# shubhamchandak94/Spring

Hardware: AMD Instinct MI355X
Metric: Mreads/s through reorder stage (higher is better)
Workload: dtype u64; 1 GPU; 100000000 x 150 bp single-end synthetic reads per GPU (uniform genome 600000000 bp, 25x coverage, 1.0% substitutions, 50% reverse-complemented), inputs resident in HBM as .dna records; reads_per_gpu=100000000, read_len=150, chains=65536, num_thr=8, parallelism=single GPU, unmatched=13958636, singletons=12720853, rounds=1984, chain_groups=2

## Files before the change

### __graft_entry__.py

```python
import os
import sys

ROOT = os.path.dirname(os.path.abspath(__file__))
for p in (ROOT, os.path.join(ROOT, "tests")):
    if p not in sys.path:
        sys.path.insert(0, p)


def build():
    from spring_amd import build as b
    lib = b.build()
    assert os.path.exists(lib)
    from oracle import pyoracle
    pyoracle.build()
    import spring_amd
    from spring_amd import _lib
    _lib.lib()


def smoke():
    import numpy as np
    import spring_amd
    from oracle import pyoracle as po
    n, L = 20000, 100
    dna = spring_amd.synth_dna_host(n, L, n * L // 25, 1, 10000)
    read, ln = po.load_dna(dna, n, L)
    for K, fused, A, PH, KA, want in ((1, 0, 1, 1, 0, po.reorder_serial(read, ln, L)), (64, 0, 1, 1, 0, po.reorder_rounds(read, ln, L, 64, 2)),
                                  (64, 3, 1, 1, 0, po.reorder_rounds(read, ln, L, 64, 2)), (64, 3, 1, 1, -1, po.reorder_rounds(read, ln, L, 64, 2)),
                                  (64, 0, 2, 1, 0, po.reorder_rounds(read, ln, L, 64, 2, alternatives=2)),
                                  (4096, 3, 1, 2, 0, po.reorder_rounds_ph(read, ln, L, 4096, 2))):
        got = spring_amd.reorder_dna(dna, n, L, spring_amd.ReorderOpts(device=0, num_chains=K, num_thr=1 if K == 1 else 2, fused=fused,
                                                                       alternatives=A, phases=PH, known_absent=KA))
        for k in ("order", "rc", "flag", "pos", "rlen", "order_s"):
            assert np.array_equal(got[k], want[k]), (K, fused, A, PH, KA, k)
    from spring_amd.encoder import EncoderStage
    with spring_amd.ReorderStage(spring_amd.ReorderOpts(device=0, num_chains=64, num_thr=2, fused=3, alternatives=1, phases=1)) as st:
        st.load_dna(dna, n, L)
        st.run()
        streams = st.streams()
        with EncoderStage(0) as enc:
            enc.encode(st)
            got = enc.streams()
    want = po.encode(read, ln, L, streams, num_thr=2)
    for k in ("seq", "pos", "noise", "noisepos", "order", "rlen", "rc", "unaligned"):
        a, b = got[k], want[k]
        assert (a == b) if isinstance(a, bytes) else np.array_equal(a, b), ("encoder", k)
    print("smoke OK: %d reads, K=1, K=64 (both round kernels) and two chain groups bit-exact vs oracle; encoder stage bit-exact (%d contigs)"
          % (n, got["num_contigs"]))


if __name__ == "__main__":
    build()
    if "--smoke" in sys.argv:
        smoke()
```

### include/spring_reorder.h

```cpp
#ifndef SPRING_REORDER_H_
#define SPRING_REORDER_H_

#include <stddef.h>
#include <stdint.h>

#ifdef __cplusplus
extern "C" {
#endif

#define SPRING_REORDER_E_ARG (-1)
#define SPRING_REORDER_E_IO (-2)
#define SPRING_REORDER_E_HIP (-3)
#define SPRING_REORDER_E_STATE (-4)

typedef struct spring_reorder_ctx spring_reorder_ctx;

typedef struct {
  int32_t device;
  uint32_t num_chains;
  int32_t num_thr;
  int32_t collect_stats;
  int32_t time_search;
  int32_t force_literal_update;
  int32_t rounds_per_sync;
// ... 2 lines not shown
  int32_t seed_wide;
  int32_t tab_scale;
  int32_t search_wpb;
  int32_t dbg_search_lds;
  int32_t dbg_apply_lds;
  int32_t fused;
  int32_t deep_bins;
  int32_t num_devices;
  int32_t devices[8];
  int32_t mg_host_transport;
  int32_t table_mode;
  int32_t plan0[6];
  int32_t plan1[6];
  int32_t long_min;
  int32_t long_blocks;
  int32_t debug;
  int32_t long_split;
  int32_t entry_flags;
  int32_t out_writers;
  int32_t alternatives;
  int32_t phases;
  int32_t known_absent;
  int32_t sort_prefix_bits;
} spring_reorder_opts;

typedef struct {
  uint64_t n_reads, n_matched, n_single, unmatched;
  uint64_t probes, keyok, cands, hits, iterations, rounds, lost;
  uint64_t numkeys[2], dict_numreads[2];
  double ms_unpack, ms_dict, ms_chains, ms_finalize, ms_total;
  double ms_search_kernel;
  uint64_t search_launches;
  uint64_t device_bytes;
  double ms_exchange, ms_resolve_mark;
  uint64_t chains;
  uint64_t deep_pool;
  uint64_t long_searches;
  uint64_t table_minz;
  uint64_t table_marked_lines;
  uint64_t long_splits;
  uint64_t alternatives;
  uint64_t phases;
  double ms_search_busy;
  uint64_t sort_prefix_bits;
  uint64_t sort_repaired_runs;
  uint64_t sort_full_sorts;
  uint64_t sort_long_runs;
  uint64_t sort_list_overflows;
} spring_reorder_stats;

void spring_reorder_default_opts(spring_reorder_opts *o);
const char *spring_reorder_last_error(void);
void spring_reorder_trim_pool(void);

int spring_reorder_run(const char *temp_dir, uint32_t max_readlen, int32_t num_thr, int32_t paired_end,
                       uint32_t num_reads_clean_0, uint32_t num_reads_clean_1,
                       const spring_reorder_opts *opts );

int spring_reorder_create(spring_reorder_ctx **ctx, const spring_reorder_opts *opts);
void spring_reorder_destroy(spring_reorder_ctx *ctx);

int spring_reorder_load_dna(spring_reorder_ctx *ctx, const uint8_t *dna, size_t nbytes, uint32_t n,
                            uint32_t max_readlen);

int spring_reorder_load_dna_device(spring_reorder_ctx *ctx, const void *d_dna, size_t nbytes, uint32_t n,
                                   uint32_t max_readlen, int32_t fixed_len);

int spring_reorder_build_dict(spring_reorder_ctx *ctx);

int spring_reorder_run_chains(spring_reorder_ctx *ctx);
int spring_reorder_auto_chains(spring_reorder_ctx *ctx, uint32_t *chains, int32_t *deep);
// ... 74 lines not shown
```

### spring_amd/_lib.py

```python
import ctypes as C
import os

HERE = os.path.dirname(os.path.abspath(__file__))
LIB_PATH = os.environ.get("SPRING_AMD_LIB") or os.path.join(HERE, "lib", "libspring_reorder_hip.so")

EXPORTS = [
    "spring_reorder_default_opts", "spring_reorder_last_error", "spring_reorder_trim_pool", "spring_reorder_run", "spring_reorder_create",
    "spring_reorder_destroy", "spring_reorder_load_dna", "spring_reorder_load_dna_device",
    "spring_reorder_build_dict", "spring_reorder_run_chains", "spring_reorder_auto_chains", "spring_reorder_finalize",
    "spring_reorder_mg_begin", "spring_reorder_mg_search", "spring_reorder_mg_slice", "spring_reorder_mg_slices",
    "spring_reorder_mg_apply",
    "spring_reorder_mg_end", "spring_reorder_mg_exchange_virtual", "spring_reorder_debug_check_seed_state",
    "spring_mg_rccl_unique_id", "spring_mg_comm_create_rccl", "spring_mg_comm_create_host", "spring_mg_comm_destroy",
    "spring_reorder_mg_run",
    "spring_reorder_get_stats", "spring_reorder_download", "spring_reorder_tid_split", "spring_reorder_emit_dna",
    "spring_reorder_dict_lookup", "spring_reorder_download_reads", "spring_synth_dna_bytes",
    "spring_reorder_load_fastq", "spring_reorder_fastq_N",
    "spring_order_invert_se", "spring_order_invert_pe", "spring_order_correct", "spring_order_pe_encode",
    "spring_fastq_reorder",
    "spring_synth_dna_host", "spring_synth_genome_host", "spring_synth_dna_device", "spring_reorder_load_synth", "spring_reorder_download_dna",
    "spring_encoder_create", "spring_encoder_destroy", "spring_encoder_set_split_tables", "spring_encoder_encode_reorder", "spring_encoder_download",
    "spring_encoder_download_seq_packed", "spring_encoder_get_info", "spring_reorder_encode_run", "spring_encoder_encode_host", "spring_encoder_run",
]

# ... 1 lines not shown
    "spring_streams_create", "spring_streams_destroy", "spring_streams_from_encoder", "spring_streams_from_host",
    "spring_streams_download", "spring_streams_get_info", "spring_streams_run",
]
STREAMS_NUM = 9

DECODE_EXPORTS = [
    "spring_decode_create", "spring_decode_destroy", "spring_decode_seq_from_encoder", "spring_decode_seq_from_host",
    "spring_decode_seq_from_files", "spring_decode_from_streams", "spring_decode_from_host", "spring_decode_from_files",
    "spring_decode_download", "spring_decode_get_info",
]


class Opts(C.Structure):
    _fields_ = [("device", C.c_int32), ("num_chains", C.c_uint32), ("num_thr", C.c_int32),
                ("collect_stats", C.c_int32), ("time_search", C.c_int32), ("force_literal_update", C.c_int32),
                ("rounds_per_sync", C.c_int32), ("long_budget", C.c_int32),
                ("first_shifts", C.c_int32), ("seed_wide", C.c_int32), ("tab_scale", C.c_int32),
                ("search_wpb", C.c_int32), ("dbg_search_lds", C.c_int32), ("dbg_apply_lds", C.c_int32),
                ("fused", C.c_int32), ("deep_bins", C.c_int32),
                ("num_devices", C.c_int32), ("devices", C.c_int32 * 8), ("mg_host_transport", C.c_int32),
                ("table_mode", C.c_int32), ("plan0", C.c_int32 * 6), ("plan1", C.c_int32 * 6), ("long_min", C.c_int32),
                ("long_blocks", C.c_int32), ("debug", C.c_int32), ("long_split", C.c_int32), ("entry_flags", C.c_int32),
                ("out_writers", C.c_int32), ("alternatives", C.c_int32), ("phases", C.c_int32), ("known_absent", C.c_int32),
                ("sort_prefix_bits", C.c_int32)]


class FastqInfo(C.Structure):
    _fields_ = [("num_reads", C.c_uint32 * 2), ("num_reads_clean", C.c_uint32 * 2), ("num_reads_N", C.c_uint32 * 2),
                ("max_readlen", C.c_uint32), ("pad", C.c_uint32), ("ms_device", C.c_double)]


class EncoderInfo(C.Structure):
    _fields_ = ([(k, C.c_uint64) for k in ("n_aligned", "n_total", "seq_len", "noise_bytes", "n_noisepos",
                                           "unaligned_bytes", "len_unaligned", "num_contigs")]
                + [(k, C.c_uint32) for k in ("matched_s", "matched_N", "align_passes", "max_bin")]
                + [("ms_device", C.c_double), ("ms_phase", C.c_double * 8)])

    def asdict(self):
        d = {}
        for k, _ in self._fields_:
            v = getattr(self, k)
            d[k] = list(v) if hasattr(v, "__len__") else v
        return d


class StreamsInfo(C.Structure):
    _fields_ = ([("num_units", C.c_uint64), ("num_blocks", C.c_uint64), ("bytes", C.c_uint64 * STREAMS_NUM),
# ... 14 lines not shown
                + [(k, C.c_uint64) for k in ("n_aligned", "n_unaligned", "pos_escapes")]
                + [("ms_device", C.c_double), ("ms_file", C.c_double)])

    def asdict(self):
        d = {}
        for k, _ in self._fields_:
            v = getattr(self, k)
            d[k] = list(v) if hasattr(v, "__len__") else v
        return d


class Stats(C.Structure):
    _fields_ = ([(k, C.c_uint64) for k in ("n_reads", "n_matched", "n_single", "unmatched", "probes", "keyok",
                                          "cands", "hits", "iterations", "rounds", "lost")]
                + [("numkeys", C.c_uint64 * 2), ("dict_numreads", C.c_uint64 * 2)]
                + [(k, C.c_double) for k in ("ms_unpack", "ms_dict", "ms_chains", "ms_finalize", "ms_total",
                                             "ms_search_kernel")]
                + [("search_launches", C.c_uint64), ("device_bytes", C.c_uint64),
                   ("ms_exchange", C.c_double), ("ms_resolve_mark", C.c_double), ("chains", C.c_uint64),
                   ("deep_pool", C.c_uint64), ("long_searches", C.c_uint64),
                   ("table_minz", C.c_uint64), ("table_marked_lines", C.c_uint64), ("long_splits", C.c_uint64), ("alternatives", C.c_uint64), ("phases", C.c_uint64),
                   ("ms_search_busy", C.c_double),
                   ("sort_prefix_bits", C.c_uint64), ("sort_repaired_runs", C.c_uint64), ("sort_full_sorts", C.c_uint64),
                   ("sort_long_runs", C.c_uint64), ("sort_list_overflows", C.c_uint64)])

    def asdict(self):
        d = {}
        for k, _ in self._fields_:
            v = getattr(self, k)
            d[k] = list(v) if hasattr(v, "__len__") else v
        return d


MG_ALLGATHER_FN = C.CFUNCTYPE(C.c_int, C.c_void_p, C.c_size_t, C.c_size_t, C.c_size_t, C.c_void_p)

_lib = None


def lib():
    global _lib
    if _lib is not None:
        return _lib
    if not os.path.exists(LIB_PATH):
        raise RuntimeError(
            "spring_amd: %s is missing. Build it with `python -m spring_amd.build` "
            "(or __graft_entry__.build()); there is no CPU fallback." % LIB_PATH)
    L = C.CDLL(LIB_PATH)
# ... 103 lines not shown
```

### spring_amd/csrc/reorder_device.h

```cpp
#ifndef SPRING_REORDER_DEVICE_H_
#define SPRING_REORDER_DEVICE_H_

#include <hip/hip_runtime.h>
#include <stdint.h>

namespace sr {

constexpr int MAX_READ_LEN = 511;
constexpr int MAX_SEARCH = 1000;
constexpr int THRESH = 4;
constexpr uint32_t DEEP_BIN = 16;
constexpr uint32_t MID_BIN = 64;
constexpr uint32_t BIG_BIN = 256;
constexpr uint32_t CHUNK = 64;
constexpr uint32_t MARK_BLOCK = 256;
constexpr uint32_t MC_WAVES_PER_BLOCK = MARK_BLOCK / 4 + 3;
constexpr int UBLK_SHIFT = 12;
constexpr int LDS_PAD = 10;
constexpr int LDS_LIMBS = 16 + 2 * LDS_PAD;

enum { MODE_SEARCH = 0, MODE_NEED_SEED = 1 };
enum { PROP_NONE = 0, PROP_MATCH = 1, PROP_SEED = 2, PROP_FRESH = 3  };
enum { PK_NONE = 0, PK_MATCH = 1, PK_SEED = 2, PK_NOSEED = 4, PK_DONE = 5 };
constexpr unsigned long long PK_CURSOR_BIT = 1ull << 35;
constexpr unsigned long long PK_WILLNEED_BIT = 1ull << 36;
constexpr int PK_ALT_SHIFT = 37;
constexpr uint32_t ALT_MAX_READS = (1u << 27) - 1;
constexpr uint32_t ALT_KEY = 1u << 28;

struct __attribute__((aligned(16))) ChainHot {
  long long ref_pos;
  int32_t ref_len;
  uint32_t e_slot;
  uint32_t prev, first_rid;
  uint32_t n_emit, n_single;
  uint32_t s_slot;
  uint32_t num_reads_thr, num_unmatched_past;
  uint32_t prop_rid;
  union {
    struct {
      uint32_t done : 1, prev_unmatched : 1, left_search : 1, stop_searching : 1;
      uint32_t mode : 1, retrying : 1, finishing : 1, cursor_writer : 1;
      uint32_t cnt_buf : 1;
      uint32_t cnt_wide : 1;
      uint32_t prop_kind : 2;
      uint32_t prop_rev : 3;
      uint32_t prop_shift : 9;
    };
    uint32_t flags;
  };
  uint32_t alt1;
  uint32_t pad[2];
};
static_assert(sizeof(ChainHot) == 64, "ChainHot must be one 64-byte line");

struct __attribute__((aligned(64))) Chain {
  ChainHot h;
  uint64_t ref[16];
  uint64_t revref[16];
  uint64_t st_probes, st_keyok, st_cands, st_iter, st_lost, st_hits, n_unmatched, st_long ;
#ifdef SR_PHASE_TIMING
  uint64_t pt[64];
#endif
};
#ifndef SR_PHASE_TIMING
static_assert(sizeof(Chain) == 384, "Chain layout");
#endif

struct Globals {
  long long cursor;
  uint32_t alive;
  uint32_t e_alloc;
  uint32_t s_alloc;
  uint32_t pad;
  long long cursor_b;
};

struct TabView {
  const uint4 *buck;
  int bshift;
  int minz;
  int lshift;
};
// ... 19 lines not shown
  int plan[2][6];
  int seed_wide;
  int deep_bins;
  int search_wpb;
  int dbg_search_lds, dbg_apply_lds;
  int wl;
  int dstart[2], dend[2];
  uint32_t numkeys[2];
  TabView tab;
  const ulonglong2 *urec[2];
  const uint32_t *ids[2];
  uint32_t *epos[2];
  uint32_t idmask;
  const ulonglong2 *sig[2];
  uint64_t *taken;
  uint32_t *ublk;
  uint32_t *resv;
  uint32_t *needy;
  uint32_t *needy_cnt;
  uint32_t *needy_cnt_next;
  int fused;
  int alts;
  int mc;
  int ka, ka_lo;
  uint32_t *ord;
  uint4 *ord_cnt;
  uint32_t *longq;
  int long_budget, long_min, long_blocks, long_part;
  uint32_t *lctl, *lparts;
  struct LongHead *lhead;
  uint2 *lbin;
  uint16_t *lbcode;
  uint32_t lbin_stride;
#ifdef SR_PHASE_TIMING
  unsigned long long *dbg;
#endif
  Globals *glob;
  long long *cursor;
  uint32_t K, c0, Ktot;
  int phases;
  uint32_t g0, Kg, g0_other, Kg_other;
  uint32_t gg0, gKg, gKg_other;
  uint32_t seed_lo, seed_hi;
  uint32_t nb_lo, nb_hi;
  const uint64_t *taken_other;
  uint32_t *won, *won_other;
// ... 90 lines not shown
```

### spring_amd/csrc/reorder_kernels.hip

```cpp
#include <cstdlib>
#include <cstring>
#include <hip/hip_runtime.h>
#include <rocprim/rocprim.hpp>

#include "reorder_device.h"
#include "synth_common.h"

namespace sr {


__device__ __forceinline__ uint64_t mix64(uint64_t x) {
  x ^= x >> 33; x *= 0xff51afd7ed558ccdull; x ^= x >> 33; x *= 0xc4ceb9fe1a85ec53ull; x ^= x >> 33;
  return x;
}

__device__ __forceinline__ void wave_sync() {
  __builtin_amdgcn_fence(__ATOMIC_SEQ_CST, "wavefront");
  __builtin_amdgcn_wave_barrier();
}

__device__ __forceinline__ int uni_i32(int v) { return __builtin_amdgcn_readfirstlane(v); }
template <class T>
__device__ __forceinline__ T *uni_ptr(T *p) {
  const uint64_t a = reinterpret_cast<uint64_t>(p);
// ... 798 lines not shown
  WaveLds *ws = &lds[wave];
  const uint32_t step = P.n / P.Ktot;
  const uint32_t seed = cid * step;
  const bool start = P.n > 0 && (cid == 0 || step > 0);
  ChainHot h;
  memset(&h, 0, sizeof(h));
  if (lane == 0) {
    P.e_chunk[li] = make_uint2(li, 0u);
    P.s_chunk[li] = make_uint2(li, 0u);
  }
  if (!start) {
    h.done = 1;
    store_hot(c, h, lane);
    if (lane == 0 && P.prop) P.prop[cid] = (unsigned long long)PK_DONE << 32;
    return;
  }
  const int n = P.uniform_len ? P.L : (int)P.lens[seed];
  bool ovf0;
  const int Rn = wave_update_compute<NP, false>(P, li, ws, nullptr, seed, n, true, false, 0, 0, 0, false, false, ovf0, lane);
  pack_consensus(ws, Rn, lane, c);
  h.prev = seed; h.first_rid = seed; h.prev_unmatched = 1;
  h.e_slot = li * CHUNK; h.s_slot = li * CHUNK;
  h.ref_len = Rn; h.cnt_buf = 1; h.cnt_wide = 0;
  if (P.fused) h.prop_kind = PROP_FRESH;
  store_hot(c, h, lane);
  if (lane == 0) {
    c->n_unmatched = 1;
    if (P.prop) P.prop[cid] = (unsigned long long)PK_NONE << 32;
  }
}
__device__ __forceinline__ void mark_dead(const DevParams &P, uint32_t rid) {
#pragma unroll
  for (int l = 0; l < 2; l++) {
    if (!P.epos[l]) continue;
    const uint32_t e = P.epos[l][rid];
    if (e != 0xffffffffu) atomicOr(const_cast<uint32_t *>(P.ids[l]) + e, 0x80000000u);
  }
}
__global__ void k_build_epos(const uint32_t *__restrict__ ids, uint64_t m, uint32_t *__restrict__ epos) {
  const uint64_t i = (uint64_t)blockIdx.x * blockDim.x + threadIdx.x;
  if (i < m) epos[ids[i]] = (uint32_t)i;
}
void launch_build_epos(hipStream_t st, const uint32_t *ids, uint64_t m, uint32_t *epos) {
  if (m) hipLaunchKernelGGL(k_build_epos, dim3((unsigned)((m + 255) / 256)), dim3(256), 0, st, ids, m, epos);
}
__global__ void k_init_seeds(DevParams P) {
// ... 1736 lines not shown
}
__global__ void k_delay(uint32_t us) {
  const uint64_t t0 = wall_clock64();
  while (wall_clock64() - t0 < (uint64_t)us * 100u) __builtin_amdgcn_s_sleep(64);
}
__global__ void k_init_ord(DevParams P) {
  const uint32_t cid = P.gg0 + blockIdx.x * blockDim.x + threadIdx.x;
  const uint32_t blk = P.gg0 / MARK_BLOCK + blockIdx.x;
  __shared__ uint32_t s_n;
  if (threadIdx.x == 0) s_n = 0;
  __syncthreads();
  const bool local = cid < P.gg0 + P.gKg && cid - P.c0 - P.g0 < P.Kg;
  const uint64_t m = __ballot(local);
  uint32_t wbase = 0;
  if ((threadIdx.x & 63) == 0 && m) wbase = atomicAdd(&s_n, (uint32_t)__popcll(m));
  wbase = (uint32_t)__shfl((int)wbase, 0, 64);
  if (local) P.ord[(size_t)blk * MARK_BLOCK + wbase + (uint32_t)__popcll(m & ((1ull << (threadIdx.x & 63)) - 1))] = cid - P.c0;
  __syncthreads();
  if (threadIdx.x == 0) P.ord_cnt[blk] = make_uint4(0u, 0u, s_n, 0u);
}

__global__ void k_chain_summary(DevParams P, uint2 *__restrict__ sum, unsigned long long *__restrict__ tot ) {
  const uint32_t i = blockIdx.x * blockDim.x + threadIdx.x;
  uint64_t v[8] = {0, 0, 0, 0, 0, 0, 0, 0};
  if (i < P.K) {
    const Chain &c = P.chains[i];
    sum[i] = make_uint2(c.h.n_emit, c.h.n_single);
    v[0] = c.n_unmatched; v[1] = c.st_probes; v[2] = c.st_keyok; v[3] = c.st_cands; v[4] = c.st_iter; v[5] = c.st_lost; v[6] = c.st_hits; v[7] = c.st_long;
  }
#pragma unroll
  for (int k = 0; k < 8; k++) {
    const uint64_t w = wave_sum_u64(v[k]);
    if ((threadIdx.x & 63) == 0 && w) atomicAdd(&tot[k], (unsigned long long)w);
  }
}

__global__ void k_scatter_matched(DevParams P, uint64_t cap, const uint64_t *__restrict__ off_m) {
  uint64_t i = (uint64_t)blockIdx.x * blockDim.x + threadIdx.x;
  if (i >= cap) return;
  const uint2 ci = P.e_chunk[i / CHUNK];
  if (ci.x == 0xffffffffu) return;
  const uint32_t seq = ci.y + (uint32_t)(i % CHUNK);
  if (seq >= P.chains[ci.x].h.n_emit) return;
  const uint4 r = P.e_rec[i];
  const uint64_t d = off_m[ci.x] + seq;
  P.f_order[d] = r.x; P.f_rc[d] = (char)(r.y & 0xffu); P.f_flag[d] = (char)((r.y >> 8) & 0xffu);
  P.f_pos[d] = (long long)((unsigned long long)r.z | ((unsigned long long)r.w << 32));
  P.f_len[d] = P.uniform_len ? (uint16_t)P.L : P.lens[r.x];
}
__global__ void k_scatter_single(DevParams P, uint64_t cap, const uint64_t *__restrict__ off_s) {
  uint64_t i = (uint64_t)blockIdx.x * blockDim.x + threadIdx.x;
  if (i >= cap) return;
  const uint2 ci = P.s_chunk[i / CHUNK];
  if (ci.x == 0xffffffffu) return;
// ... 370 lines not shown
```

### spring_amd/csrc/reorder_pipeline.cpp

```cpp
#include <hip/hip_runtime.h>
#include <dlfcn.h>

#include <algorithm>
#include <system_error>
#include <thread>
#include <memory>
#include <atomic>
#include <chrono>
#include <cstdarg>
#include <cstdio>
#include <cstdlib>
#include <cstring>
#include <map>
#include <mutex>
#include <new>
#include <stdexcept>
#include <string>
#include <unordered_map>
#include <vector>
#include <zlib.h>

#include "reorder_device.h"
#include "reorder_internal.h"
#include "spring_reorder.h"
// ... 1388 lines not shown
  DMALLOC(P.cnt8, (size_t)K * 2 * ctx->Lpad * sizeof(uint32_t) + 64);
  const size_t cap = (size_t)n + (size_t)K * CHUNK;
  if (cap > 0xfffffff0ull) return fail(SPRING_REORDER_E_ARG, "n + K*%u exceeds the 32-bit slot space", CHUNK);
  ctx->cap = cap;
  const size_t nchunk = cap / CHUNK + 2;
  DMALLOC(P.e_rec, cap * sizeof(uint4)); DMALLOC(P.e_chunk, nchunk * sizeof(uint2));
  DMALLOC(P.s_rec, cap * 4); DMALLOC(P.s_chunk, nchunk * sizeof(uint2));
  P.mc = ctx->o.fused == 2 ? 0 : 1;
  bool ka_ok = false;
  int ka_lo = 0;
  if (P.Lpad <= 192 && ctx->o.known_absent >= 0 && !ctx->minz) {
    const int wlen = ctx->dict[0].end - ctx->dict[0].start + 1, lo = ctx->dict[0].start >> 5;
    if (wlen <= 32 && ctx->dict[1].start == ctx->dict[0].end + 1 && ctx->dict[1].end - ctx->dict[1].start + 1 == wlen &&
        2 * (ctx->L - wlen) + 2 <= 64 * (lo + 4) && 2 * ctx->dict[1].start + 2 <= 256 && lo + 4 <= 6) {
      ka_ok = true; ka_lo = lo;
    }
  }
  const uint64_t nd_ = (uint64_t)ctx->dict[0].numreads + ctx->dict[1].numreads, nk_ = (uint64_t)ctx->dict[0].numkeys + ctx->dict[1].numkeys;
  const uint32_t mc_min = P.phases == 2 ? ((ka_ok && nd_ * 100 < nk_ * 105) ? 20480u : 32768u) : 49152u;
  if (K < mc_min && ctx->o.fused != 3) P.mc = 0;
  if (64 - ctx->bshift > 32) P.mc = 0;
  P.ka = (P.mc && ka_ok) ? 1 : 0;
  P.ka_lo = P.ka ? ka_lo : 0;
  if (ctx->minz && !(fused && P.mc && !ctx->o.collect_stats && !P.deep_bins))
    return fail(SPRING_REORDER_E_ARG, "table_mode = 2 (minimizer-addressed table) is an experiment of the four-chain round kernel: "
                "shallow dictionary, at least 49152 chains or fused = 3, no work counters");
  if (!P.mc && !P.deep_bins && ctx->o.first_shifts == 0 && !ctx->user_plan0) {
    memset(P.plan[0], 0, sizeof(P.plan[0]));
    P.plan[0][0] = 8; P.plan[0][1] = 16;
  }
  P.g0 = 0; P.Kg = K; P.g0_other = 0; P.Kg_other = 0;
  P.gg0 = 0; P.gKg = Ktot; P.gKg_other = 0;
  P.seed_lo = 0; P.seed_hi = n;
  P.nb_lo = 0; P.nb_hi = (Ktot + 2047) / 2048;
  P.taken_other = nullptr; P.won = P.won_other = nullptr;
  ctx->taken2 = nullptr; ctx->resv2 = nullptr; ctx->won = nullptr;
  ctx->lb2 = spring_reorder_ctx::LongBufs();
  if (P.phases == 2) {
    DMALLOC(ctx->taken2, nwords * 8);
    DMALLOC(ctx->resv2, nn * 4);
    DMALLOC(ctx->won, (size_t)Ktot * 4);
  }
  P.prop = nullptr; P.alive_wave = nullptr; P.needy_cnt = P.needy_cnt_next = nullptr;
  ctx->cnt_buf[0] = ctx->cnt_buf[1] = nullptr;
  if (fused && P.deep_bins && ctx->o.entry_flags >= 0 && n < 0x80000000u) {
    for (int l = 0; l < 2; l++) {
// ... 827 lines not shown
    ctx->stats.ms_search_kernel = ms_round; ctx->stats.ms_search_busy = ms_round; ctx->stats.search_launches = timed_rounds;
    ctx->stats.ms_exchange = ms_xchg; ctx->stats.ms_resolve_mark = ms_mark;
  }
  if (ret) {
    const std::string keep = g_err;
    (void)hipStreamSynchronize(st);
    (void)spring_reorder_mg_end(ctx);
    g_err = keep;
    return ret;
  }
  return spring_reorder_mg_end(ctx);
}

int spring_reorder_finalize(spring_reorder_ctx *ctx) {
  if (!ctx) return fail(SPRING_REORDER_E_ARG, "ctx is NULL");
  if (ctx->stage != ST_CHAINS) return fail(SPRING_REORDER_E_STATE, "finalize: run_chains first");
  HIPCHK(hipSetDevice(ctx->dev));
  hipStream_t st = ctx->st;
  DevParams &P = ctx->P;
  const uint32_t K = ctx->K;
  const int T = ctx->o.num_thr;
  HIPCHK(hipEventRecord(ctx->ev[6], st));
  std::vector<uint2> hs(std::max<uint32_t>(K, 1));
  unsigned long long htot[8] = {0, 0, 0, 0, 0, 0, 0, 0};
  Globals g;
  {
    uint2 *d_sum = nullptr;
    unsigned long long *d_tot = nullptr;
    DMALLOC(d_sum, (size_t)std::max<uint32_t>(K, 1) * sizeof(uint2));
    DMALLOC(d_tot, 64);
    HIPCHK(hipMemsetAsync(d_tot, 0, 64, st));
    launch_chain_summary(st, P, d_sum, d_tot);
    HIPCHK(hipGetLastError());
    if (K) HIPCHK(hipMemcpyAsync(hs.data(), d_sum, (size_t)K * sizeof(uint2), hipMemcpyDeviceToHost, st));
    HIPCHK(hipMemcpyAsync(htot, d_tot, 64, hipMemcpyDeviceToHost, st));
    HIPCHK(hipMemcpyAsync(&g, P.glob, sizeof(g), hipMemcpyDeviceToHost, st));
    HIPCHK(hipStreamSynchronize(st));
    ctx->dfree(d_sum); ctx->dfree(d_tot);
  }
#ifdef SR_PHASE_TIMING
  std::vector<Chain> hc(K);
  if (K) HIPCHK(hipMemcpy(hc.data(), P.chains, (size_t)K * sizeof(Chain), hipMemcpyDeviceToHost));
#endif
  std::vector<uint64_t> off_m(K), off_s(K);
  ctx->tid_off.assign(T + 1, 0);
  ctx->tid_off_s.assign(T + 1, 0);
  uint64_t am = 0, as = 0;
  spring_reorder_stats &s = ctx->stats;
  s.unmatched = s.probes = s.keyok = s.cands = s.iterations = s.lost = s.hits = 0;
  ctx->tid_mid.assign(T, 0);
  ctx->tid_mid_s.assign(T, 0);
  for (int t = 0; t < T; t++) {
    ctx->tid_off[t] = am;
    ctx->tid_off_s[t] = as;
    for (int g = 0; g < 2; g++) {
      const auto &a = ctx->grp[g];
      if (g == 1) { ctx->tid_mid[t] = am; ctx->tid_mid_s[t] = as; }
      if (!a.Kg) continue;
// ... 29 lines not shown
    fprintf(stderr, "\n");
    std::vector<std::pair<unsigned long long, uint32_t>> top;
    for (uint32_t i = 0; i < K; i++) {
      unsigned long long t = 0;
      for (int k = 0; k < 32; k++) t += hc[i].pt[k];
      top.push_back({t, i});
    }
    std::partial_sort(top.begin(), top.begin() + std::min<size_t>(3, top.size()), top.end(), std::greater<>());
    for (size_t j = 0; j < std::min<size_t>(3, top.size()); j++) {
      fprintf(stderr, "[phase] chain %u: %llu clocks:", top[j].second, top[j].first);
      for (int k = 0; k < 32; k++)
        if (hc[top[j].second].pt[32 + k]) fprintf(stderr, " %d:%u/%u", k, hc[top[j].second].pt[k], hc[top[j].second].pt[32 + k]);
      fprintf(stderr, "\n");
    }
  }
#endif
  if ((!ctx->mg && am + as != ctx->n) || am + as > ctx->n || g.e_alloc > ctx->cap + CHUNK || g.s_alloc > ctx->cap + CHUNK)
    return fail(SPRING_REORDER_E_STATE, "internal: emission counts do not add up (%llu+%llu vs n=%u, alloc %u/%u cap %llu)",
                (unsigned long long)am, (unsigned long long)as, ctx->n, g.e_alloc, g.s_alloc,
                (unsigned long long)ctx->cap);
  ctx->nrec = am;
  ctx->nsing = as;
  s.n_reads = ctx->n; s.n_matched = am; s.n_single = as;
  const size_t nm = std::max<uint64_t>(am, 1), ns = std::max<uint64_t>(as, 1);
  DMALLOC(P.f_order, nm * 4); DMALLOC(P.f_rc, nm); DMALLOC(P.f_flag, nm); DMALLOC(P.f_pos, nm * 8);
  DMALLOC(P.f_len, nm * 2); DMALLOC(P.f_order_s, ns * 4);
  uint64_t *d_off_m = nullptr, *d_off_s = nullptr;
  DMALLOC(d_off_m, (size_t)K * 8);
  DMALLOC(d_off_s, (size_t)K * 8);
  HIPCHK(hipMemcpyAsync(d_off_m, off_m.data(), (size_t)K * 8, hipMemcpyHostToDevice, st));
  HIPCHK(hipMemcpyAsync(d_off_s, off_s.data(), (size_t)K * 8, hipMemcpyHostToDevice, st));
  launch_scatter(st, P, am ? ctx->cap : 0, as ? ctx->cap : 0, d_off_m, d_off_s);
  HIPCHK(hipGetLastError());
  HIPCHK(hipEventRecord(ctx->ev[7], st));
  HIPCHK(hipStreamSynchronize(st));
  s.long_splits = 0;
  if (P.lctl) {
    uint32_t ns = 0;
    HIPCHK(hipMemcpy(&ns, P.lctl + 3, 4, hipMemcpyDeviceToHost));
    s.long_splits = ns;
    if (P.phases == 2 && ctx->lb2.lctl) {
      HIPCHK(hipMemcpy(&ns, ctx->lb2.lctl + 3, 4, hipMemcpyDeviceToHost));
      s.long_splits += ns;
    }
  }
  ctx->dfree(d_off_m); ctx->dfree(d_off_s);
// ... 148 lines not shown
```

### spring_amd/csrc/reorder_round_mc.h

```cpp
#ifndef SPRING_REORDER_ROUND_MC_H_
#define SPRING_REORDER_ROUND_MC_H_

namespace mc {

constexpr int G = 16;
constexpr int CPW = 64 / G;

template <int NQ, bool KA>
struct GLds {
  static constexpr int WMAX = NQ <= 3 ? 6 : 16;
  static constexpr int PAD = NQ <= 3 ? 4 : LDS_PAD;
  static constexpr int LIMBS = WMAX + 2 * PAD;
  static constexpr int MZ = NQ <= 3 && !KA ? 164 : 4;
  uint64_t refs[2][LIMBS];
  uint64_t rd[WMAX + 2];
  uint64_t nref[WMAX];
  union {
    uint8_t pres[128];
    uint64_t ka[2][KA ? LIMBS : 2];
  };
  uint32_t best;
  uint32_t pad[3];
  uint32_t mz[MZ];
};
// ... 12 lines not shown
#pragma unroll
  for (int o = 1; o < G; o <<= 1) {
    const int t = __shfl_up(v, o, G);
    if (gl >= o) v += t;
  }
  return v;
}
__device__ __forceinline__ uint32_t gballot(bool p, int lane) {
  return (uint32_t)(__ballot(p) >> (lane & ~(G - 1))) & 0xffffu;
}
__device__ __forceinline__ uint64_t gshfl_u64(uint64_t v, int src) {
  const uint32_t lo = __shfl((uint32_t)v, src, G), hi = __shfl((uint32_t)(v >> 32), src, G);
  return ((uint64_t)hi << 32) | lo;
}

__device__ __forceinline__ uint32_t rd_bits8(const uint64_t *rd, int bitpos) {
  const int bp = bitpos + 64, li = bp >> 6, off = bp & 63;
  uint64_t v = rd[li] >> off;
  if (off > 56) v |= rd[li + 1] << (64 - off);
  return (uint32_t)v & 0xffu;
}

typedef uint32_t u32x4a_t __attribute__((ext_vector_type(4), aligned(4)));

template <int NQ, bool KA>
__device__ __forceinline__ int update_mc(const DevParams &P, uint32_t li, GLds<NQ, KA> &S, uint32_t rid, int n, bool reset,
                                         bool rev, int shift, int R, int cb, bool cur_wide, bool out_wide,
                                         bool &overflow, int gl, int *o_src = nullptr, int *o_cpy = nullptr, bool *o_alias = nullptr) {
  const int M = P.L, W = P.W;
  const int4 *__restrict__ cur = P.cnt + ((uint64_t)li * 2 + cb) * P.Lpad;
  int4 *__restrict__ nxt = P.cnt + ((uint64_t)li * 2 + (cb ^ 1)) * P.Lpad;
  const uint32_t *__restrict__ cur8 = P.cnt8 + ((uint64_t)li * 2 + cb) * P.Lpad;
  uint32_t *__restrict__ nxt8 = P.cnt8 + ((uint64_t)li * 2 + (cb ^ 1)) * P.Lpad;
  int hiP, cpy_hi, src_off, add_lo, add_hi, Rn, d = 0;
  bool alias = false;
  if (reset) { hiP = M; cpy_hi = 0; src_off = 0; add_lo = 0; add_hi = n; Rn = n; }
  else if (!rev) { Rn = max(R - shift, n); hiP = Rn; cpy_hi = R - shift; src_off = shift; add_lo = 0; add_hi = n; }
  else if (n - shift >= R) { Rn = n; hiP = n; cpy_hi = R; src_off = 0; add_lo = 0; add_hi = n; d = n - shift - R; alias = d > 0; }
  else if (R + shift <= M) { Rn = R + shift; hiP = Rn; cpy_hi = R; src_off = 0; add_lo = R - n + shift; add_hi = Rn; }
  else { Rn = M; hiP = M; cpy_hi = M - shift; src_off = R + shift - M; add_lo = M - n; add_hi = M; }
  const bool fast = !alias && !cur_wide && !out_wide;
  if (o_src) { *o_src = src_off; *o_cpy = cpy_hi; *o_alias = alias; }

  const uint64_t myl = gl < W ? P.reads[(uint64_t)rid * P.S + gl] : 0ull;
  u32x4a_t old[NQ];
#pragma unroll
  for (int k = 0; k < NQ; k++) {
    const int p0 = 4 * (gl + G * k);
    old[k] = (u32x4a_t)(0u);
    if (fast && p0 < cpy_hi) old[k] = *reinterpret_cast<const u32x4a_t *>(cur8 + p0 + src_off);
  }
  if (gl < GLds<NQ, KA>::WMAX) S.rd[1 + gl] = myl;
  wave_sync();
  const uint64_t *rd = S.rd;

  bool ovf = false;
#pragma unroll
  for (int k = 0; k < NQ; k++) {
    const int q = gl + G * k, p0 = 4 * q;
    if (p0 >= P.Lpad) continue;
    uint32_t codes = 0;
    if (fast) {
      const int i0 = p0 - add_lo;
      uint32_t b8 = 0;
      if (i0 > -4 && i0 < n) {
        if (!rev) b8 = rd_bits8(rd, 2 * i0);
        else {
          const uint32_t x = ~rd_bits8(rd, 2 * (n - 4 - i0)) & 0xffu;
          b8 = ((x & 3u) << 6) | ((x & 0xcu) << 2) | ((x >> 2) & 0xcu) | (x >> 6);
        }
      }
      u32x4a_t t4;
#pragma unroll
      for (int e = 0; e < 4; e++) {
        const int p = p0 + e;
        uint32_t t = p < cpy_hi ? old[k][e] : 0u;
        const uint32_t code = (b8 >> (2 * e)) & 3u;
        uint32_t cdx = code;
        if (p >= add_lo && p < add_hi) {
          const uint32_t sh = (0x10081800u >> (8 * code)) & 31u;
          ovf = ovf || ((t >> sh) & 255u) == 255u;
          t += 1u << sh;
        }
        if (p >= hiP) t = 0u;
        t4[e] = t;
        if (!reset) {
          const uint32_t ka = ((t & 255u) << 2) | 3u, kc = (((t >> 8) & 255u) << 2) | 2u,
                         kt = (((t >> 16) & 255u) << 2) | 1u, kg = (t >> 24) << 2;
          const uint32_t ind = 3u - (max(max(ka, kc), max(kt, kg)) & 3u);
          cdx = (0x1320u >> (4 * ind)) & 3u;
        }
        if (p < Rn) codes |= cdx << (2 * e);
      }
      if (p0 < hiP) *reinterpret_cast<uint4 *>(nxt8 + p0) = make_uint4(t4[0], t4[1], t4[2], t4[3]);
    } else {
#define MC_LOAD_CNT(I) (cur_wide ? cur[(I)] : unpack8(cur8[(I)]))
      for (int e = 0; e < 4; e++) {
        const int p = p0 + e;
        if (p >= hiP) continue;
        int4 t = make_int4(0, 0, 0, 0);
        int code = 0;
        if (!alias) {
          if (p < cpy_hi) t = MC_LOAD_CNT(p + src_off);
          if (p >= add_lo && p < add_hi) {
            code = cur_base(rd + 1, p - add_lo, n, rev);
            add_hot(t, cidx_of_code(code));
          }
        } else {
          if (p >= d && p < n - shift) {
            t = MC_LOAD_CNT(p % d);
            for (int qq = p % d + d; qq <= p; qq += d) add_hot(t, cidx_of_code(cur_base(rd + 1, qq, n, rev)));
          } else {
            add_hot(t, cidx_of_code(cur_base(rd + 1, p, n, rev)));
          }
        }
        if (out_wide) nxt[p] = t; else nxt8[p] = pack8(t);
        ovf = ovf || max(max(t.x, t.y), max(t.z, t.w)) > 255;
        if (p < Rn) codes |= (uint32_t)(reset ? code : argmax_code(t)) << (2 * e);
      }
#undef MC_LOAD_CNT
    }
    if (q < 8 * GLds<NQ, KA>::WMAX) reinterpret_cast<uint8_t *>(S.nref)[q] = (uint8_t)codes;
  }
  overflow = gballot(ovf, (int)threadIdx.x) != 0;
  return Rn;
}

template <int NQ, bool KA>
__device__ __forceinline__ void commit_consensus(const DevParams &P, GLds<NQ, KA> &S, Chain *c, int R, int gl) {
  constexpr int LDS_PAD = GLds<NQ, KA>::PAD;
  wave_sync();
  const bool in = gl < P.W;
  const uint64_t limb = in ? S.nref[gl] : 0ull;
  if (gl < GLds<NQ, KA>::WMAX) S.refs[0][LDS_PAD + gl] = limb;
  if (in) c->ref[gl] = limb;
  wave_sync();
  uint64_t rl = 0;
  if (in && 32 * gl < R) {
    const uint64_t w = lds_window(S.refs[0] + LDS_PAD, 2 * (R - 32 - 32 * gl));
// ... 106 lines not shown

template <int NQ, bool KA>
__device__ __forceinline__ bool apply_mc(const DevParams &P, Chain *c, uint32_t cid, uint32_t li, ChainHot &h, GLds<NQ, KA> &S, int gl) {
  const int kind = h.prop_kind;
  if (kind == PROP_FRESH) return true;
  if (h.finishing) {
    if (h.prev_unmatched) emit_single_mc(P, h, li, h.prev, gl);
    h.done = 1; h.finishing = 0;
    store_hot(c, h, gl);
    return false;
  }
  const uint32_t owner = kind != PROP_NONE ? P.resv[h.prop_rid] : cid;
  const bool fail_path = kind == PROP_NONE && h.mode == MODE_SEARCH;
  bool do_upd = false, ureset = false, urev = false;
  uint32_t urid = 0;
  int ushift = 0;
  if (kind == PROP_MATCH) { do_upd = true; urid = h.prop_rid; urev = h.prop_rev & 1; ushift = (int)h.prop_shift; }
  else if (kind == PROP_SEED) { do_upd = true; urid = h.prop_rid; ureset = true; }
  else if (fail_path && !h.left_search) { do_upd = true; urid = h.first_rid; ureset = true; urev = true; }
  int n = P.L, R_new = h.ref_len;
  const int R_old = h.ref_len;
  bool nw = false, ualias = false;
  int usrc = 0, ucpy = 0;
  if (do_upd) {
    if (!P.uniform_len) n = (int)P.lens[urid];
    R_new = update_mc<NQ, KA>(P, li, S, urid, n, ureset, urev, ushift, R_old, (int)h.cnt_buf, h.cnt_wide != 0, false, nw, gl,
                          &usrc, &ucpy, &ualias);
    if (nw) {
      bool o2;
      wave_sync();
      R_new = update_mc<NQ, KA>(P, li, S, urid, n, ureset, urev, ushift, R_old, (int)h.cnt_buf, h.cnt_wide != 0, true, o2, gl);
    }
  }
  if (owner != cid) {
    if (h.mode == MODE_SEARCH) h.retrying = 1;
    store_hot(c, h, gl, 3, 4);
    if (gl == 0) atomicAdd((unsigned long long *)&c->st_lost, 1ull);
    return true;
  }
  if (do_upd) {
    if constexpr (KA) {
      const int kmode = kind == PROP_MATCH ? (ualias ? 1 : 0) : (kind != PROP_SEED && h.prev_unmatched) ? 2 : 1;
      commit_consensus_ka<NQ, KA>(P, S, c, R_old, R_new, usrc, ucpy, kmode, gl);
    } else commit_consensus<NQ, KA>(P, S, c, R_new, gl);
    h.ref_len = R_new;
    h.cnt_buf ^= 1;
    h.cnt_wide = nw;
  }
  if (kind == PROP_MATCH) {
    const uint32_t rid = h.prop_rid;
    const int shift = ushift;
    const bool left = h.left_search;
    long long ref_pos = h.ref_pos, cur_pos;
    char rcch;
    if (!urev) {
      if (!left) { cur_pos = ref_pos + shift; ref_pos = cur_pos; }
      else { cur_pos = ref_pos + R_old - shift - n; ref_pos = ref_pos + R_old - shift - R_new; }
      rcch = left ? 'r' : 'd';
    } else {
      if (!left) { cur_pos = ref_pos + R_old + shift - n; ref_pos = ref_pos + R_old + shift - R_new; }
      else { cur_pos = ref_pos - shift; ref_pos = cur_pos; }
      rcch = left ? 'd' : 'r';
    }
    if (h.prev_unmatched) emit_rec_mc(P, h, li, h.prev, 'd', '0', 0, gl);
    emit_rec_mc(P, h, li, rid, rcch, '1', cur_pos, gl);
    h.prev_unmatched = 0; h.ref_pos = ref_pos; h.retrying = 0;
  } else if (kind == PROP_SEED) {
    const uint32_t rid = h.prop_rid;
    if (gl == 0) atomicAdd((unsigned long long *)&c->n_unmatched, 1ull);
// ... 755 lines not shown
```

### spring_amd/reorder.py

```python
import ctypes as C
from dataclasses import dataclass

import numpy as np

from . import _lib


class ReorderError(RuntimeError):
    """Raised where the reference throws std::runtime_error (call_template_functions.cpp:60)."""


@dataclass
class ReorderOpts:
    device: int = -1
    num_chains: int = 0
    num_thr: int = 1
    collect_stats: bool = False
    time_search: bool = False
    force_literal_update: bool = False
    rounds_per_sync: int = 0
    first_shifts: int = 0
    seed_wide: int = 0
    tab_scale: int = 0
    search_wpb: int = 0
    dbg_search_lds: int = 0
    dbg_apply_lds: int = 0
    fused: int = 0
    deep_bins: int = 0
    long_budget: int = 0
    devices: tuple = ()
    mg_host_transport: bool = False
    plan0: tuple = ()
    plan1: tuple = ()
    long_min: int = 0
    long_blocks: int = 0
    entry_flags: int = 0
    long_split: int = 0
    debug: bool = False
    out_writers: int = 0
    alternatives: int = 0
    table_mode: int = 0
    phases: int = 0
    known_absent: int = 0
    sort_prefix_bits: int = 0

    def to_c(self):
        o = _lib.Opts()
        _lib.lib().spring_reorder_default_opts(C.byref(o))
        o.device, o.num_chains, o.num_thr = self.device, self.num_chains, self.num_thr
        o.collect_stats, o.time_search = int(self.collect_stats), int(self.time_search)
        o.force_literal_update, o.rounds_per_sync = int(self.force_literal_update), self.rounds_per_sync
        o.first_shifts, o.seed_wide, o.tab_scale = self.first_shifts, self.seed_wide, self.tab_scale
        o.search_wpb, o.dbg_search_lds, o.dbg_apply_lds = self.search_wpb, self.dbg_search_lds, self.dbg_apply_lds
        o.fused, o.deep_bins = self.fused, self.deep_bins
        o.long_budget = self.long_budget
        if len(self.devices) > 8:
            raise ValueError("at most 8 devices")
        o.table_mode = self.table_mode
        for i, v in enumerate(tuple(self.plan0)[:6]):
            o.plan0[i] = int(v)
        for i, v in enumerate(tuple(self.plan1)[:6]):
            o.plan1[i] = int(v)
        o.long_min, o.long_blocks, o.debug = self.long_min, self.long_blocks, int(self.debug)
        o.long_split, o.entry_flags = self.long_split, self.entry_flags
        o.out_writers = self.out_writers
        o.alternatives = self.alternatives
        o.phases = self.phases
        o.known_absent = self.known_absent
        o.sort_prefix_bits = self.sort_prefix_bits
        o.num_devices = len(self.devices)
        for i, d in enumerate(self.devices):
            o.devices[i] = d
        o.mg_host_transport = int(self.mg_host_transport)
        return o


def _chk(rc):
    if rc != 0:
        raise ReorderError("%s (code %d)" % (_lib.lib().spring_reorder_last_error().decode(), rc))


class ReorderStage:

    def __init__(self, opts: ReorderOpts = None):
        self.opts = opts or ReorderOpts()
        self._L = _lib.lib()
        self._h = C.c_void_p()
        _chk(self._L.spring_reorder_create(C.byref(self._h), C.byref(self.opts.to_c())))
        self.n = 0
        self.max_readlen = 0

    def close(self):
# ... 171 lines not shown
```

Measured before the change: 333.6 Mreads/s.

## Imply count columns from reference after reset instead of storing them

Adds a compact-count mode, on by default when the fused multi-chain round kernel runs without stats or deep bins. After a chain resets, the per-position count array is not written. A flag marks the counts as implied, and the next update rebuilds the one-hot counts from the consensus reference held in LDS. A lone turn-around with no prior match copies the reference instead of running an update. This is meant to cut global count-buffer stores and loads on the many reset and single-read chain steps. The cost is extra per-element decode logic and a new header flag bit, and the probes and keyok counters are reused as new update counters.

```diff
diff --git a/__graft_entry__.py b/__graft_entry__.py
--- a/__graft_entry__.py
+++ b/__graft_entry__.py
@@ -25,14 +25,15 @@
     n, L = 20000, 100
     dna = spring_amd.synth_dna_host(n, L, n * L // 25, 1, 10000)
     read, ln = po.load_dna(dna, n, L)
-    for K, fused, A, PH, KA, want in ((1, 0, 1, 1, 0, po.reorder_serial(read, ln, L)), (64, 0, 1, 1, 0, po.reorder_rounds(read, ln, L, 64, 2)),
-                                  (64, 3, 1, 1, 0, po.reorder_rounds(read, ln, L, 64, 2)), (64, 3, 1, 1, -1, po.reorder_rounds(read, ln, L, 64, 2)),
-                                  (64, 0, 2, 1, 0, po.reorder_rounds(read, ln, L, 64, 2, alternatives=2)),
-                                  (4096, 3, 1, 2, 0, po.reorder_rounds_ph(read, ln, L, 4096, 2))):
+    for K, fused, A, PH, KA, CC, want in ((1, 0, 1, 1, 0, 0, po.reorder_serial(read, ln, L)), (64, 0, 1, 1, 0, 0, po.reorder_rounds(read, ln, L, 64, 2)),
+                                  (64, 3, 1, 1, 0, 0, po.reorder_rounds(read, ln, L, 64, 2)), (64, 3, 1, 1, -1, 0, po.reorder_rounds(read, ln, L, 64, 2)),
+                                  (64, 3, 1, 1, 0, -1, po.reorder_rounds(read, ln, L, 64, 2)),
+                                  (64, 0, 2, 1, 0, 0, po.reorder_rounds(read, ln, L, 64, 2, alternatives=2)),
+                                  (4096, 3, 1, 2, 0, 0, po.reorder_rounds_ph(read, ln, L, 4096, 2))):
         got = spring_amd.reorder_dna(dna, n, L, spring_amd.ReorderOpts(device=0, num_chains=K, num_thr=1 if K == 1 else 2, fused=fused,
-                                                                       alternatives=A, phases=PH, known_absent=KA))
+                                                                       alternatives=A, phases=PH, known_absent=KA, compact_counts=CC))
         for k in ("order", "rc", "flag", "pos", "rlen", "order_s"):
-            assert np.array_equal(got[k], want[k]), (K, fused, A, PH, KA, k)
+            assert np.array_equal(got[k], want[k]), (K, fused, A, PH, KA, CC, k)
     from spring_amd.encoder import EncoderStage
     with spring_amd.ReorderStage(spring_amd.ReorderOpts(device=0, num_chains=64, num_thr=2, fused=3, alternatives=1, phases=1)) as st:
         st.load_dna(dna, n, L)
diff --git a/include/spring_reorder.h b/include/spring_reorder.h
--- a/include/spring_reorder.h
+++ b/include/spring_reorder.h
@@ -48,6 +48,7 @@
   int32_t phases;
   int32_t known_absent;
   int32_t sort_prefix_bits;
+  int32_t compact_counts;
 } spring_reorder_opts;
 
 typedef struct {
@@ -73,6 +74,7 @@
   uint64_t sort_full_sorts;
   uint64_t sort_long_runs;
   uint64_t sort_list_overflows;
+  uint64_t upd_implied, upd_compact, upd_byte, upd_wide;
 } spring_reorder_stats;
 
 void spring_reorder_default_opts(spring_reorder_opts *o);
diff --git a/spring_amd/_lib.py b/spring_amd/_lib.py
--- a/spring_amd/_lib.py
+++ b/spring_amd/_lib.py
@@ -47,7 +47,7 @@
                 ("table_mode", C.c_int32), ("plan0", C.c_int32 * 6), ("plan1", C.c_int32 * 6), ("long_min", C.c_int32),
                 ("long_blocks", C.c_int32), ("debug", C.c_int32), ("long_split", C.c_int32), ("entry_flags", C.c_int32),
                 ("out_writers", C.c_int32), ("alternatives", C.c_int32), ("phases", C.c_int32), ("known_absent", C.c_int32),
-                ("sort_prefix_bits", C.c_int32)]
+                ("sort_prefix_bits", C.c_int32), ("compact_counts", C.c_int32)]
 
 
 class FastqInfo(C.Structure):
@@ -108,7 +108,8 @@
                    ("table_minz", C.c_uint64), ("table_marked_lines", C.c_uint64), ("long_splits", C.c_uint64), ("alternatives", C.c_uint64), ("phases", C.c_uint64),
                    ("ms_search_busy", C.c_double),
                    ("sort_prefix_bits", C.c_uint64), ("sort_repaired_runs", C.c_uint64), ("sort_full_sorts", C.c_uint64),
-                   ("sort_long_runs", C.c_uint64), ("sort_list_overflows", C.c_uint64)])
+                   ("sort_long_runs", C.c_uint64), ("sort_list_overflows", C.c_uint64),
+                   ("upd_implied", C.c_uint64), ("upd_compact", C.c_uint64), ("upd_byte", C.c_uint64), ("upd_wide", C.c_uint64)])
 
     def asdict(self):
         d = {}
diff --git a/spring_amd/csrc/reorder_device.h b/spring_amd/csrc/reorder_device.h
--- a/spring_amd/csrc/reorder_device.h
+++ b/spring_amd/csrc/reorder_device.h
@@ -46,6 +46,7 @@
       uint32_t prop_kind : 2;
       uint32_t prop_rev : 3;
       uint32_t prop_shift : 9;
+      uint32_t cnt_implied : 1;
     };
     uint32_t flags;
   };
@@ -58,7 +59,9 @@
   ChainHot h;
   uint64_t ref[16];
   uint64_t revref[16];
-  uint64_t st_probes, st_keyok, st_cands, st_iter, st_lost, st_hits, n_unmatched, st_long ;
+  union { uint64_t st_probes, st_upd_wide; };
+  union { uint64_t st_keyok, st_upd_implied; };
+  uint64_t st_cands, st_iter, st_lost, st_hits, n_unmatched, st_long ;
 #ifdef SR_PHASE_TIMING
   uint64_t pt[64];
 #endif
@@ -124,6 +127,7 @@
   int fused;
   int alts;
   int mc;
+  int colfmt;
   int ka, ka_lo;
   uint32_t *ord;
   uint4 *ord_cnt;
diff --git a/spring_amd/csrc/reorder_kernels.hip b/spring_amd/csrc/reorder_kernels.hip
--- a/spring_amd/csrc/reorder_kernels.hip
+++ b/spring_amd/csrc/reorder_kernels.hip
@@ -844,6 +844,7 @@
   h.prev = seed; h.first_rid = seed; h.prev_unmatched = 1;
   h.e_slot = li * CHUNK; h.s_slot = li * CHUNK;
   h.ref_len = Rn; h.cnt_buf = 1; h.cnt_wide = 0;
+  h.cnt_implied = P.colfmt == 2;
   if (P.fused) h.prop_kind = PROP_FRESH;
   store_hot(c, h, lane);
   if (lane == 0) {
@@ -2626,14 +2627,15 @@
 
 __global__ void k_chain_summary(DevParams P, uint2 *__restrict__ sum, unsigned long long *__restrict__ tot ) {
   const uint32_t i = blockIdx.x * blockDim.x + threadIdx.x;
-  uint64_t v[8] = {0, 0, 0, 0, 0, 0, 0, 0};
+  uint64_t v[12] = {0, 0, 0, 0, 0, 0, 0, 0, 0, 0, 0, 0};
   if (i < P.K) {
     const Chain &c = P.chains[i];
     sum[i] = make_uint2(c.h.n_emit, c.h.n_single);
     v[0] = c.n_unmatched; v[1] = c.st_probes; v[2] = c.st_keyok; v[3] = c.st_cands; v[4] = c.st_iter; v[5] = c.st_lost; v[6] = c.st_hits; v[7] = c.st_long;
+    if (P.colfmt) { v[1] = v[2] = 0; v[8] = c.st_upd_implied; v[11] = c.st_upd_wide; }
   }
 #pragma unroll
-  for (int k = 0; k < 8; k++) {
+  for (int k = 0; k < 12; k++) {
     const uint64_t w = wave_sum_u64(v[k]);
     if ((threadIdx.x & 63) == 0 && w) atomicAdd(&tot[k], (unsigned long long)w);
   }
diff --git a/spring_amd/csrc/reorder_pipeline.cpp b/spring_amd/csrc/reorder_pipeline.cpp
--- a/spring_amd/csrc/reorder_pipeline.cpp
+++ b/spring_amd/csrc/reorder_pipeline.cpp
@@ -1434,6 +1434,7 @@
   if (64 - ctx->bshift > 32) P.mc = 0;
   P.ka = (P.mc && ka_ok) ? 1 : 0;
   P.ka_lo = P.ka ? ka_lo : 0;
+  P.colfmt = (fused && P.mc && !ctx->o.collect_stats && !P.deep_bins) ? (ctx->o.compact_counts >= 0 ? 2 : 1) : 0;
   if (ctx->minz && !(fused && P.mc && !ctx->o.collect_stats && !P.deep_bins))
     return fail(SPRING_REORDER_E_ARG, "table_mode = 2 (minimizer-addressed table) is an experiment of the four-chain round kernel: "
                 "shallow dictionary, at least 49152 chains or fused = 3, no work counters");
@@ -2307,18 +2308,18 @@
   const int T = ctx->o.num_thr;
   HIPCHK(hipEventRecord(ctx->ev[6], st));
   std::vector<uint2> hs(std::max<uint32_t>(K, 1));
-  unsigned long long htot[8] = {0, 0, 0, 0, 0, 0, 0, 0};
+  unsigned long long htot[12] = {0, 0, 0, 0, 0, 0, 0, 0, 0, 0, 0, 0};
   Globals g;
   {
     uint2 *d_sum = nullptr;
     unsigned long long *d_tot = nullptr;
     DMALLOC(d_sum, (size_t)std::max<uint32_t>(K, 1) * sizeof(uint2));
-    DMALLOC(d_tot, 64);
-    HIPCHK(hipMemsetAsync(d_tot, 0, 64, st));
+    DMALLOC(d_tot, sizeof(htot));
+    HIPCHK(hipMemsetAsync(d_tot, 0, sizeof(htot), st));
     launch_chain_summary(st, P, d_sum, d_tot);
     HIPCHK(hipGetLastError());
     if (K) HIPCHK(hipMemcpyAsync(hs.data(), d_sum, (size_t)K * sizeof(uint2), hipMemcpyDeviceToHost, st));
-    HIPCHK(hipMemcpyAsync(htot, d_tot, 64, hipMemcpyDeviceToHost, st));
+    HIPCHK(hipMemcpyAsync(htot, d_tot, sizeof(htot), hipMemcpyDeviceToHost, st));
     HIPCHK(hipMemcpyAsync(&g, P.glob, sizeof(g), hipMemcpyDeviceToHost, st));
     HIPCHK(hipStreamSynchronize(st));
     ctx->dfree(d_sum); ctx->dfree(d_tot);
@@ -2394,6 +2395,8 @@
   ctx->nrec = am;
   ctx->nsing = as;
   s.n_reads = ctx->n; s.n_matched = am; s.n_single = as;
+  s.upd_implied = htot[8]; s.upd_compact = 0; s.upd_wide = htot[11];
+  s.upd_byte = P.colfmt ? am - (s.unmatched - as) - s.upd_implied - s.upd_wide : 0;
   const size_t nm = std::max<uint64_t>(am, 1), ns = std::max<uint64_t>(as, 1);
   DMALLOC(P.f_order, nm * 4); DMALLOC(P.f_rc, nm); DMALLOC(P.f_flag, nm); DMALLOC(P.f_pos, nm * 8);
   DMALLOC(P.f_len, nm * 2); DMALLOC(P.f_order_s, ns * 4);
diff --git a/spring_amd/csrc/reorder_round_mc.h b/spring_amd/csrc/reorder_round_mc.h
--- a/spring_amd/csrc/reorder_round_mc.h
+++ b/spring_amd/csrc/reorder_round_mc.h
@@ -58,11 +58,17 @@
 }
 
 typedef uint32_t u32x4a_t __attribute__((ext_vector_type(4), aligned(4)));
+__device__ __forceinline__ int4 hot_of_ref(const uint64_t *sref, int i) {
+  int4 t = make_int4(0, 0, 0, 0);
+  add_hot(t, cidx_of_code((int)((sref[i >> 5] >> (2 * (i & 31))) & 3ull)));
+  return t;
+}
 
 template <int NQ, bool KA>
 __device__ __forceinline__ int update_mc(const DevParams &P, uint32_t li, GLds<NQ, KA> &S, uint32_t rid, int n, bool reset,
                                          bool rev, int shift, int R, int cb, bool cur_wide, bool out_wide,
-                                         bool &overflow, int gl, int *o_src = nullptr, int *o_cpy = nullptr, bool *o_alias = nullptr) {
+                                         bool &overflow, int gl, int *o_src = nullptr, int *o_cpy = nullptr, bool *o_alias = nullptr,
+                                         bool cur_imp = false) {
   const int M = P.L, W = P.W;
   const int4 *__restrict__ cur = P.cnt + ((uint64_t)li * 2 + cb) * P.Lpad;
   int4 *__restrict__ nxt = P.cnt + ((uint64_t)li * 2 + (cb ^ 1)) * P.Lpad;
@@ -76,6 +82,8 @@
   else if (R + shift <= M) { Rn = R + shift; hiP = Rn; cpy_hi = R; src_off = 0; add_lo = R - n + shift; add_hi = Rn; }
   else { Rn = M; hiP = M; cpy_hi = M - shift; src_off = R + shift - M; add_lo = M - n; add_hi = M; }
   const bool fast = !alias && !cur_wide && !out_wide;
+  const bool no_store = reset && P.colfmt == 2;
+  const uint64_t *sref0 = S.refs[0] + GLds<NQ, KA>::PAD;
   if (o_src) { *o_src = src_off; *o_cpy = cpy_hi; *o_alias = alias; }
 
   const uint64_t myl = gl < W ? P.reads[(uint64_t)rid * P.S + gl] : 0ull;
@@ -84,8 +92,19 @@
   for (int k = 0; k < NQ; k++) {
     const int p0 = 4 * (gl + G * k);
     old[k] = (u32x4a_t)(0u);
-    if (fast && p0 < cpy_hi) old[k] = *reinterpret_cast<const u32x4a_t *>(cur8 + p0 + src_off);
-  }
+    if (fast && !cur_imp && p0 < cpy_hi) old[k] = *reinterpret_cast<const u32x4a_t *>(cur8 + p0 + src_off);
+  }
+#ifdef SR_EXP_COL2
+  const uint32_t *__restrict__ cur8x = reinterpret_cast<const uint32_t *>(cur);
+  uint32_t *__restrict__ nxt8x = reinterpret_cast<uint32_t *>(nxt);
+  u32x4a_t oldx[NQ];
+#pragma unroll
+  for (int k = 0; k < NQ; k++) {
+    const int p0 = 4 * (gl + G * k);
+    oldx[k] = (u32x4a_t)(0u);
+    if (fast && !cur_imp && p0 < cpy_hi) oldx[k] = *reinterpret_cast<const u32x4a_t *>(cur8x + p0 + src_off);
+  }
+#endif
   if (gl < GLds<NQ, KA>::WMAX) S.rd[1 + gl] = myl;
   wave_sync();
   const uint64_t *rd = S.rd;
@@ -106,11 +125,16 @@
           b8 = ((x & 3u) << 6) | ((x & 0xcu) << 2) | ((x >> 2) & 0xcu) | (x >> 6);
         }
       }
+      uint32_t c8 = 0;
+      if (cur_imp && p0 < cpy_hi) c8 = (uint32_t)lds_window(sref0, 2 * (p0 + src_off));
       u32x4a_t t4;
+#ifdef SR_EXP_COL2
+      asm volatile("" ::"v"(oldx[k][0]), "v"(oldx[k][1]), "v"(oldx[k][2]), "v"(oldx[k][3]));
+#endif
 #pragma unroll
       for (int e = 0; e < 4; e++) {
         const int p = p0 + e;
-        uint32_t t = p < cpy_hi ? old[k][e] : 0u;
+        uint32_t t = p < cpy_hi ? (cur_imp ? 1u << ((0x10081800u >> (8 * ((c8 >> (2 * e)) & 3u))) & 31u) : old[k][e]) : 0u;
         const uint32_t code = (b8 >> (2 * e)) & 3u;
         uint32_t cdx = code;
         if (p >= add_lo && p < add_hi) {
@@ -128,9 +152,12 @@
         }
         if (p < Rn) codes |= cdx << (2 * e);
       }
-      if (p0 < hiP) *reinterpret_cast<uint4 *>(nxt8 + p0) = make_uint4(t4[0], t4[1], t4[2], t4[3]);
+      if (p0 < hiP && !no_store) *reinterpret_cast<uint4 *>(nxt8 + p0) = make_uint4(t4[0], t4[1], t4[2], t4[3]);
+#ifdef SR_EXP_COL2
+      if (p0 < hiP && !no_store) *reinterpret_cast<uint4 *>(nxt8x + p0) = make_uint4(t4[0], t4[1], t4[2], t4[3]);
+#endif
     } else {
-#define MC_LOAD_CNT(I) (cur_wide ? cur[(I)] : unpack8(cur8[(I)]))
+#define MC_LOAD_CNT(I) (cur_imp ? hot_of_ref(sref0, (I)) : cur_wide ? cur[(I)] : unpack8(cur8[(I)]))
       for (int e = 0; e < 4; e++) {
         const int p = p0 + e;
         if (p >= hiP) continue;
@@ -150,7 +177,7 @@
             add_hot(t, cidx_of_code(cur_base(rd + 1, p, n, rev)));
           }
         }
-        if (out_wide) nxt[p] = t; else nxt8[p] = pack8(t);
+        if (no_store) {} else if (out_wide) nxt[p] = t; else nxt8[p] = pack8(t);
         ovf = ovf || max(max(t.x, t.y), max(t.z, t.w)) > 255;
         if (p < Rn) codes |= (uint32_t)(reset ? code : argmax_code(t)) << (2 * e);
       }
@@ -303,14 +330,19 @@
   const int R_old = h.ref_len;
   bool nw = false, ualias = false;
   int usrc = 0, ucpy = 0;
-  if (do_upd) {
+  const bool imp = P.colfmt == 2, cur_imp = imp && h.cnt_implied;
+  const bool lone_turn = imp && fail_path && !h.left_search && h.prev_unmatched;
+  if (lone_turn) {
+    if (gl < GLds<NQ, KA>::WMAX) S.nref[gl] = S.refs[1][GLds<NQ, KA>::PAD + gl];
+  } else if (do_upd) {
     if (!P.uniform_len) n = (int)P.lens[urid];
     R_new = update_mc<NQ, KA>(P, li, S, urid, n, ureset, urev, ushift, R_old, (int)h.cnt_buf, h.cnt_wide != 0, false, nw, gl,
-                          &usrc, &ucpy, &ualias);
+                          &usrc, &ucpy, &ualias, cur_imp);
     if (nw) {
       bool o2;
       wave_sync();
-      R_new = update_mc<NQ, KA>(P, li, S, urid, n, ureset, urev, ushift, R_old, (int)h.cnt_buf, h.cnt_wide != 0, true, o2, gl);
+      R_new = update_mc<NQ, KA>(P, li, S, urid, n, ureset, urev, ushift, R_old, (int)h.cnt_buf, h.cnt_wide != 0, true, o2, gl,
+                            nullptr, nullptr, nullptr, cur_imp);
     }
   }
   if (owner != cid) {
@@ -325,7 +357,15 @@
       commit_consensus_ka<NQ, KA>(P, S, c, R_old, R_new, usrc, ucpy, kmode, gl);
     } else commit_consensus<NQ, KA>(P, S, c, R_new, gl);
     h.ref_len = R_new;
-    h.cnt_buf ^= 1;
+    if (imp && ureset) h.cnt_implied = 1;
+    else {
+      if (kind == PROP_MATCH && gl == 0) {
+        if (cur_imp) atomicAdd((unsigned long long *)&c->st_upd_implied, 1ull);
+        else if (h.cnt_wide) atomicAdd((unsigned long long *)&c->st_upd_wide, 1ull);
+      }
+      h.cnt_buf ^= 1;
+      h.cnt_implied = 0;
+    }
     h.cnt_wide = nw;
   }
   if (kind == PROP_MATCH) {
diff --git a/spring_amd/reorder.py b/spring_amd/reorder.py
--- a/spring_amd/reorder.py
+++ b/spring_amd/reorder.py
@@ -43,6 +43,7 @@
     phases: int = 0
     known_absent: int = 0
     sort_prefix_bits: int = 0
+    compact_counts: int = 0
 
     def to_c(self):
         o = _lib.Opts()
@@ -68,6 +69,7 @@
         o.phases = self.phases
         o.known_absent = self.known_absent
         o.sort_prefix_bits = self.sort_prefix_bits
+        o.compact_counts = self.compact_counts
         o.num_devices = len(self.devices)
         for i, d in enumerate(self.devices):
             o.devices[i] = d
```

Result: faster. 338.4 Mreads/s (median of 6 runs) (+1.4%).
